# roncapat/UNIGE-TASI-path-planners

Hardware: AMD Instinct MI355X
Metric: grid cells updated/sec (full plan + 100 replans), 4096^2 map (higher is better)
Workload: dtype f32

## Files before the change

### unige-tasi-path-planners_amd/csrc/ufm_region.h

```cpp

#ifndef UFM_REGION_IDLE_SLEEP_RAISE
#define UFM_REGION_IDLE_SLEEP_RAISE 8
#endif
#ifndef UFM_REGION_PRIO
#define UFM_REGION_PRIO 2
#endif
#if UFM_REGION_PRIO
#define UFM_REGION_SETPRIO(x) __builtin_amdgcn_s_setprio(x)
#else
#define UFM_REGION_SETPRIO(x) do {} while (0)
#endif
#ifndef UFM_REGION_IDLE_SLEEP
#define UFM_REGION_IDLE_SLEEP 8
#endif
constexpr int RTMAX = 128 / T;
constexpr int RN = RTMAX * T;
constexpr int RP = RN + 8;
constexpr int RCP = RN + 4;
constexpr int RBP = RN;
constexpr int TP = T / 4;
constexpr int RPW = RTMAX * TP / 4;
constexpr int RWW = (RPW * RPW + 31) / 32;
constexpr int RFRAME = 4 * RTMAX + 4;

struct RegionJob {
    ReplanBegin rb;
    DevDyn dyn;
    int tx0, ty0, ntx, nty;
    int k_lower;
    unsigned int seq;
    int max_sweeps;
    int debug;
    float slack;
    float delta;
    int map;
    int batch;
    const uint8_t *psrc[4];
};
constexpr int RJOBS = 8;
struct RegionJobs { int n; RegionJob j[RJOBS]; };

__device__ __forceinline__ int prio_read_fresh(const DevParams &P, int qz, int kk, int gt) {
    const unsigned long long v = __hip_atomic_load(&P.prio[(size_t)(qz * 2 + (kk & 1)) * P.NT + gt], __ATOMIC_RELAXED, __HIP_MEMORY_SCOPE_AGENT);
    return (int)(v >> 32) == 0x7FFFFFFF - kk ? (int)(unsigned int)v : INFBITS;
}

struct RegionShared {
    int wake[16][RWW];
    int ever[16][RWW];
    int renew[16][RWW];
    int tbp[RTMAX * RTMAX];
    int seed[16][RWW];
    int defer[2][16][RWW];
    int dprio[2][RTMAX * RTMAX];
    int tflag[RTMAX * RTMAX];
    int traised[RTMAX * RTMAX];
    int actL[RFRAME], actR[RFRAME];
    int soff[4];
    float sdist[4];
    float B0, rbound;
    float theta;
    float Bgate;
    int rmin;
    float Bsub;
    int swas[4];
    int idle, giveup, again, any_start_in;
    unsigned long long sweeps;
    int expanded;
    int m_r, m_l, done;
    int dkey;
    int dbg[8];
    int dbg2[8];
    unsigned long long tstamp[12];
};

__device__ __forceinline__ float region_start_key(const float *Gs, const RegionShared &S) {
    if (!S.any_start_in) return S.B0;
    float b = 0.0f;
#pragma unroll
    for (int i = 0; i < 4; ++i) {
        const int o = S.soff[i];
        if (o < 0) continue;
        const float g = Gs[o];
        if (g < INFINITY) b = fmaxf(b, g + S.sdist[i]);
    }
    return b > 0.0f ? b : INFINITY;
}

__device__ __forceinline__ float region_lower_bound(const float *Gs, const RegionShared &S) {
    if (!S.any_start_in) return S.B0;
    float b = 0.0f;
    bool pending = false;
#pragma unroll
    for (int i = 0; i < 4; ++i) {
        const int o = S.soff[i];
        if (o < 0) continue;
        const float g = Gs[o];
        if (g < INFINITY) b = fmaxf(b, g + S.sdist[i]);
        else if (S.swas[i]) pending = true;
    }
    if (pending) return fmaxf(b, S.rbound);
    return b > 0.0f ? b : INFINITY;
}

template <int ALGOF, int MODE>
__device__ void region_phase(const DevParams &P, const RegionJob &J, float *Gs, const uint8_t *Cb, uint8_t *Bb, RegionShared &S,
                             int thr, float hm, int focused, int goal_lx, int goal_ly) {
    constexpr int ALGO = algo_of(ALGOF);
    constexpr bool FOLLOW = (ALGOF & ALGO_FOLLOW_INFO) != 0;
    constexpr bool BPRAISE = MODE == MODE_RAISE && (!is_dfm<ALGO> || FOLLOW);
    const int tid = threadIdx.x, w = wave_index16(tid >> 6), lane = tid & 63;
    const int q = lane & 3, nd = lane >> 2;
    const int nprow = J.ntx * TP, npcol = J.nty * TP;
    unsigned long long wake_sel = 0ull;
    if (lane < 9) {
        const int dr = lane / 3 - 1, dc = lane % 3 - 1;
        wake_sel = ~0ull;
        if (dr < 0) wake_sel &= 0x000000000000FFFFull; else if (dr > 0) wake_sel &= 0xFFFF000000000000ull;
        if (dc < 0) wake_sel &= 0x000F000F000F000Full; else if (dc > 0) wake_sel &= 0xF000F000F000F000ull;
    }
    const int colour = ((nd >> 2) & 1) | ((nd & 1) << 1);
    const bool wt_lane = lane < 9;
    const int wt_dr = wt_lane ? lane / 3 - 1 : 0, wt_dc = wt_lane ? lane % 3 - 1 : 0;
    const int wt_ar = (w >> 2) + wt_dr, wt_ac = (w & 3) + wt_dc;
    const int wt_wave = ((wt_ar & 3) << 2) | (wt_ac & 3), wt_di = (wt_ar >> 2) * RPW + (wt_ac >> 2);
    const float sx = J.rb.sb.sx, sy = J.rb.sb.sy;
    const int rx0 = J.tx0 * T, ry0 = J.ty0 * T;
    int budget = J.max_sweeps;
    unsigned int my_sweeps = 0;
    auto cost_at = [=](int r, int c) { const int b = Cb[r * RCP + c]; return b >= thr ? INFINITY : (float)b; };
    const int so0 = __builtin_amdgcn_readfirstlane(S.soff[0]), so1 = __builtin_amdgcn_readfirstlane(S.soff[1]);
    const int so2 = __builtin_amdgcn_readfirstlane(S.soff[2]), so3 = __builtin_amdgcn_readfirstlane(S.soff[3]);
    const bool dbg_nogate = (J.debug & 1) != 0, dbg_count = (J.debug & 2) != 0;
    const float Bphase = (MODE == MODE_LOWER) ? S.Bgate : INFINITY;
    const float rb_phase = S.rbound + J.slack;
    const int nwords = min(RWW, (((nprow + 3) / 4 - 1) * RPW + (npcol + 3) / 4 + 31) / 32);
    UFM_REGION_SETPRIO(UFM_REGION_PRIO);
    for (;;) {
        bool took = false;
        bool vote = __hip_atomic_load(&S.giveup, __ATOMIC_RELAXED, __HIP_MEMORY_SCOPE_WORKGROUP) != 0;
        for (int wd = 0; wd < nwords && !vote; ++wd) {
            if (__hip_atomic_load(&S.wake[w][wd], __ATOMIC_RELAXED, __HIP_MEMORY_SCOPE_WORKGROUP) == 0) continue;
            int bits = 0;
            if (lane == 0) bits = atomicExch(&S.wake[w][wd], 0);
            bits = __builtin_amdgcn_readfirstlane(bits);
            if (!bits) continue;
            if (MODE == MODE_RAISE && lane == 0) S.ever[w][wd] |= bits;
            int seedbits = 0;
            if (BPRAISE) seedbits = __builtin_amdgcn_readfirstlane(S.seed[w][wd]) & bits;
            while (bits) {
                const int j = __ffs(bits) - 1;
                if (budget <= 0) {
                    if (lane == 0) {
                        __hip_atomic_fetch_or(&S.wake[w][wd], bits, __ATOMIC_RELAXED, __HIP_MEMORY_SCOPE_WORKGROUP);
                        __hip_atomic_store(&S.giveup, 1, __ATOMIC_RELAXED, __HIP_MEMORY_SCOPE_WORKGROUP);
                    }
                    vote = true;
                    break;
                }
                bits &= bits - 1;
                took = true;
                const int idx = wd * 32 + j;
                const int pr = (idx / RPW) * 4 + (w >> 2), pc = (idx % RPW) * 4 + (w & 3);
                if (pr >= nprow || pc >= npcol) continue;
                const int lx = pr * 4 + (nd >> 2), ly = pc * 4 + (nd & 3);
                const bool arith = BPRAISE && ((seedbits >> j) & 1);
                QuadConsts<ALGO> C;
                if (!BPRAISE || arith) C.load_at(cost_at, lx, ly, q, RP);
                float *ctr = Gs + (lx + 1) * RP + ly + 1;
                uint8_t *bpp = Bb + lx * RBP + ly;
                const int bpb = BPRAISE ? *bpp : BP_NONE;
                const int bqc = bpb >> 3, bsx = (bqc & 2) ? RP : -RP, bsy = (bqc & 1) ? 1 : -1;
                int bo1 = (bpb & 4) ? bsy : bsx, bo2 = bsx + bsy;
                if constexpr (is_dfm<ALGO>) dfm_bp_offsets<RP>(bpb, bo1, bo2);
                const bool bd1 = bpb & 1, bd2 = bpb & 2;
                const bool bnone = is_dfm<ALGO> && bpb == BP_NONE;
                const bool goal = (lx == goal_lx) & (ly == goal_ly);
                const int npr = pr + wt_dr, npc = pc + wt_dc, ni = idx + wt_di;
                const bool wt_ok = wt_lane & ((unsigned)npr < (unsigned)nprow) & ((unsigned)npc < (unsigned)npcol);
                const int nwave = wt_wave, nword = wt_ok ? (ni >> 5) : -1, nbit = 1 << (ni & 31);
                float hd = 0.0f;
                if (hm != 0.0f) {
                    const float x0 = (float)(rx0 + pr * 4), x1 = x0 + 3.0f, y0 = (float)(ry0 + pc * 4), y1 = y0 + 3.0f;
                    const float dx = fmaxf(fmaxf(x0 - sx, sx - x1), 0.0f), dy = fmaxf(fmaxf(y0 - sy, sy - y1), 0.0f);
                    hd = hm * hypotf(dx, dy) * 0.999f;
                }
                const int tl = (pr / TP) * J.nty + (pc / TP);
                const float B = Bphase;
                const int my_off = (lx + 1) * RP + ly + 1;
                const bool is_start = (my_off == so0) | (my_off == so1) | (my_off == so2) | (my_off == so3);
                const float rb = (MODE == MODE_RAISE && S.traised[tl]) ? INFINITY : rb_phase;
                asm volatile("" ::: "memory");
                float g = ctr[0];
                if (dbg_count && MODE == MODE_LOWER) {
                    const int sx_ = (q & 2) ? RP : -RP, sy_ = (q & 1) ? 1 : -1;
                    const bool fin = (g < INFINITY) | (ctr[sx_] < INFINITY) | (ctr[sy_] < INFINITY) | (ctr[sx_ + sy_] < INFINITY);
                    if (__builtin_amdgcn_ballot_w64(fin) == 0ull && lane == 0) atomicAdd(&S.dbg2[1], 1);
                }
                float dmin = INFINITY;
                float rmin_l = INFINITY;
                bool again = true, pch = false;
                [[maybe_unused]] bool held_last = false;
                [[maybe_unused]] float nv_last = INFINITY;
                [[maybe_unused]] const bool gate_free = is_start || B == INFINITY || dbg_nogate;
                unsigned long long chg = 0ull;
                int cnt = 0;
                for (int b = 0; b < 16 && again; ++b) {
                    asm volatile("" ::: "memory");
                    float nv;
                    if constexpr (BPRAISE) {
                        if (arith && b == 0) nv = quad_min(eval_quad_bp<ALGO, RP>(ctr, q, C, bpb));
                        else { const float p1 = ctr[bo1], p2 = ctr[bo2]; nv = ((bd1 && p1 == INFINITY) || (bd2 && p2 == INFINITY) || bnone) ? INFINITY : g; }
                    }
                    else nv = quad_min(eval_quad<ALGO, RP>(ctr, q, C));
                    if (goal) nv = 0.0f;
                    bool want, gate, doit;
                    if (MODE == MODE_LOWER) {
                        want = (nv != g);
                        gate = (nv + hd < B) || gate_free;
                        doit = want && gate && ((nv < g) || (colour == (cnt & 3)));
                        held_last = want && !gate; nv_last = nv;
                    } else {
                        if (is_dfm<ALGO>) want = (g < INFINITY) && (nv > g) && ((nv == INFINITY) || (__float_as_int(nv) - __float_as_int(g) > 8));
                        else want = (g < INFINITY) && (nv > g);
                        gate = !(g > rb) || dbg_nogate;
                        doit = want && gate;
                        if (want && !gate) dmin = fminf(dmin, g);
                        rmin_l = doit ? fminf(rmin_l, g) : rmin_l;
                        nv = INFINITY;
                    }
                    if (doit && q == 0) ctr[0] = nv;
                    const float gn = doit ? nv : g;
                    const unsigned long long mask = __builtin_amdgcn_ballot_w64(doit);
                    const unsigned long long wanted = __builtin_amdgcn_ballot_w64(want && gate);
                    g = gn;
                    pch |= mask != 0ull;
                    chg |= mask;
                    UFM_SWEEP_FENCE();
                    if ((mask & wake_sel) != 0ull && nword >= 0 && lane != 4)
                        __hip_atomic_fetch_or(&S.wake[nwave][nword], nbit, __ATOMIC_RELAXED, __HIP_MEMORY_SCOPE_WORKGROUP);
                    ++cnt;
                    again = wanted != 0ull;
                }
                budget -= cnt; my_sweeps += cnt;
                if (pch && lane == 0) S.tflag[tl] = 1;
                if (MODE == MODE_LOWER && held_last) dmin = nv_last;
                if ((chg & wake_sel) != 0ull && nword >= 0) __hip_atomic_fetch_or(&S.renew[nwave][nword], nbit, __ATOMIC_RELAXED, __HIP_MEMORY_SCOPE_WORKGROUP);
                if (BPRAISE && arith) {
                    const unsigned long long held = __builtin_amdgcn_ballot_w64(dmin < INFINITY);
                    if (lane == 0 && held == 0ull) S.seed[w][wd] &= ~(1 << j);
                }
                if (MODE == MODE_RAISE && rmin_l < INFINITY && q == 0) { atomicMin(&S.rmin, __float_as_int(rmin_l)); S.traised[tl] = 1; }
                if (dbg_count && lane == 0) { atomicAdd(&S.dbg[MODE == MODE_LOWER ? 5 : 4], 1); atomicAdd(&S.dbg[MODE == MODE_LOWER ? 7 : 6], cnt); if (!pch) atomicAdd(&S.dbg2[MODE == MODE_LOWER ? 0 : 2], 1); }
                if (again && lane == 0) __hip_atomic_fetch_or(&S.wake[w][wd], 1 << j, __ATOMIC_RELAXED, __HIP_MEMORY_SCOPE_WORKGROUP);
                if (dmin < INFINITY && q == 0) {
                    atomicAdd(&S.dbg[MODE == MODE_LOWER ? 0 : 1], 1);
                    atomicMin(&S.dprio[MODE == MODE_LOWER ? 0 : 1][tl], __float_as_int(dmin));
                    if (MODE == MODE_LOWER) atomicMin(&S.dkey, __float_as_int(dmin + hd));
                    __hip_atomic_fetch_or(&S.defer[MODE == MODE_LOWER ? 0 : 1][w][wd], 1 << j, __ATOMIC_RELAXED, __HIP_MEMORY_SCOPE_WORKGROUP);
                }
            }
        }
        if (took && !vote) continue;
        if (!vote) {
            if (lane == 0) atomicAdd(&S.idle, 1);
            UFM_REGION_SETPRIO(0);
            for (;;) {
                __builtin_amdgcn_s_sleep(BPRAISE ? UFM_REGION_IDLE_SLEEP_RAISE : UFM_REGION_IDLE_SLEEP);
                const int idle_now = __hip_atomic_load(&S.idle, __ATOMIC_RELAXED, __HIP_MEMORY_SCOPE_WORKGROUP);
                const int gave_up_now = __hip_atomic_load(&S.giveup, __ATOMIC_RELAXED, __HIP_MEMORY_SCOPE_WORKGROUP);
                int any = 0;
#pragma unroll
                for (int wd = 0; wd < RWW; ++wd) any |= __hip_atomic_load(&S.wake[w][wd], __ATOMIC_RELAXED, __HIP_MEMORY_SCOPE_WORKGROUP);
                if (idle_now >= 16 || gave_up_now != 0) { vote = true; break; }
                if (any) { if (lane == 0) atomicSub(&S.idle, 1); break; }
            }
            UFM_REGION_SETPRIO(UFM_REGION_PRIO);
            if (!vote) continue;
        }
        __syncthreads();
        int mine = 0;
#pragma unroll
        for (int wd = 0; wd < RWW; ++wd) mine |= __hip_atomic_load(&S.wake[w][wd], __ATOMIC_RELAXED, __HIP_MEMORY_SCOPE_WORKGROUP);
        const int work = __syncthreads_or(mine != 0);
        const int gave_up = __hip_atomic_load(&S.giveup, __ATOMIC_RELAXED, __HIP_MEMORY_SCOPE_WORKGROUP);
        if (gave_up || !work) break;
        if (tid == 0) S.idle = 0;
        __syncthreads();
    }
    UFM_REGION_SETPRIO(0);
    if (lane == 0 && my_sweeps) atomicAdd(&S.sweeps, (unsigned long long)my_sweeps);
    __syncthreads();
    if (tid == 0) S.idle = 0;
    __syncthreads();
}

template <int ALGOF>
__global__ __launch_bounds__(NTHR) void k_replan_region(DevParams P, RegionJobs JS, DevCounters *host, unsigned int *flag) {
    constexpr int ALGO = algo_of(ALGOF);
    __shared__ float Gs[(RN + 2) * RP];
    __shared__ uint8_t Cb[(RN + 1) * RCP];
    __shared__ __attribute__((aligned(16))) uint8_t Bb[RN * RBP];
    __shared__ RegionShared S;
    __shared__ int s_last;
#ifdef UFM_REGION_NG0
    constexpr int NG0 = UFM_REGION_NG0;
#else
    constexpr int NG0 = (46 * 1024) / (TT * 4);
#endif
    __shared__ float G0c[NG0 * TT];
    __shared__ int s_wbl[RTMAX * RTMAX];
    __shared__ int s_nwb;
    __shared__ uint8_t s_pmask[4096];
    __shared__ int s_simd[16];
    __shared__ unsigned long long s_tb[8];
    constexpr bool CELLS = is_dfm<ALGO>;
    constexpr int COFF = CELLS ? 0 : 1;
    const int tid = threadIdx.x;
    const RegionJob &J = JS.j[blockIdx.x];
    const int m = J.map, gt0 = m * P.NTm;
    const int ntl = J.ntx * J.nty;
    const int nty_magic = (65536 + J.nty - 1) / J.nty;
    const int rx0 = J.tx0 * T, ry0 = J.ty0 * T, rnx = J.ntx * T, rny = J.nty * T;

    const unsigned long long t_begin = wall_clock64();
#define STAMP(k) do { if (tid == 0 && (J.debug & 2)) s_tb[k] = wall_clock64(); } while (0)
    STAMP(0);
    if ((tid & 63) == 0 && (J.debug & 2)) s_simd[tid >> 6] = (int)__builtin_amdgcn_s_getreg((1 << 11) | (4 << 6) | 4);
    const float hm = J.dyn.hm;
    const int thr = J.dyn.thr, focused = J.dyn.focused;
    int r_first = -1;
    for (int r = J.rb.nrect - 1; r >= 0; --r) if (J.psrc[r]) r_first = r;
    const bool one_fused = J.rb.nrect == 1 && r_first == 0 && !J.batch;
    int pb0[4] = {0, 0, 0, 0};
    if (r_first >= 0) {
        const int n0 = J.rb.rect[r_first][3] * J.rb.rect[r_first][4];
#pragma unroll
        for (int c = 0; c < 4; ++c) { const int e = tid + c * NTHR; if (e < n0) pb0[c] = J.psrc[r_first][e]; }
    }
    float sg = INFINITY;
    int se_x = -1, se_y = -1;
    {
        const int e = tid == 0 ? J.rb.sb.start[0] : (tid == 1 ? J.rb.sb.start[1] : (tid == 2 ? J.rb.sb.start[2] : (tid == 3 ? J.rb.sb.start[3] : -1)));
        if (e >= 0) { se_x = e / P.EY; se_y = e - se_x * P.EY; sg = P.G[gaddr(P, m, se_x, se_y)]; }
    }
    const int n_pending = P.ctr->scount;
    const int goal_x = P.goal[2 * m], goal_y = P.goal[2 * m + 1];
    STAMP(1);
    const int wv = __builtin_amdgcn_readfirstlane(tid >> 6), ln = tid & 63;
    {
        const int crow = rnx + COFF, ccol = rny + COFF;
        constexpr int KP = (RN + 64) / 64, KR = (RN + 16) / 16;
        const uint8_t *cbase = P.cost + (size_t)m * P.cstride;
        uint8_t cv[KP * KR];
#pragma unroll
        for (int j = 0; j < KP; ++j) {
            const int c = j * 64 + ln, cy = ry0 + c - COFF;
            const bool cok = c < ccol && cy >= 0 && cy < P.W;
#pragma unroll
            for (int k = 0; k < KR; ++k) {
                const int r = wv + 16 * k, cx = rx0 + r - COFF;
                cv[j * KR + k] = 255;
                if (j * 64 < ccol && r < crow && cx >= 0 && cx < P.L && cok) cv[j * KR + k] = cbase[(size_t)cx * P.W + cy];
            }
        }
        constexpr int CPT = TT / 256, KT = RTMAX * RTMAX * CPT / 16;
        float4 gv[KT];
        unsigned int bv[KT];
#pragma unroll
        for (int k = 0; k < KT; ++k) {
            const int pc = wv + 16 * k, tl = pc / CPT;
            if (tl >= ntl) continue;
            const int ti = (tl * nty_magic) >> 16, tj = tl - ti * J.nty, v = (pc - tl * CPT) * 64 + ln;
            const size_t gt = (size_t)(gt0 + (J.tx0 + ti) * P.TY + J.ty0 + tj);
            gv[k] = reinterpret_cast<const float4 *>(P.G + gt * TT)[v];
            bv[k] = reinterpret_cast<const unsigned int *>(P.bp + gt * TT)[v];
        }
        static_assert(4 * RN + 4 <= NTHR, "one frame element per thread");
        float fv = INFINITY;
        int fo = -1;
        if (tid < 2 * (rny + 2) + 2 * rnx) {
            int hx, hy;
            if (tid < rny + 2) { hx = -1; hy = tid - 1; }
            else if (tid < 2 * (rny + 2)) { hx = rnx; hy = tid - (rny + 2) - 1; }
            else if (tid < 2 * (rny + 2) + rnx) { hx = tid - 2 * (rny + 2); hy = -1; }
            else { hx = tid - 2 * (rny + 2) - rnx; hy = rny; }
            const int x = rx0 + hx, y = ry0 + hy;
            fo = (hx + 1) * RP + hy + 1;
            if (x >= 0 && y >= 0 && x < P.TX * T && y < P.TY * T) fv = P.G[gaddr(P, m, x, y)];
        }
        STAMP(7);
#pragma unroll
        for (int j = 0; j < KP; ++j) {
            const int c = j * 64 + ln;
#pragma unroll
            for (int k = 0; k < KR; ++k) {
                const int r = wv + 16 * k;
                if (j * 64 < ccol && r < crow && c < ccol) Cb[r * RCP + c] = cv[j * KR + k];
            }
        }
#pragma unroll
        for (int k = 0; k < KT; ++k) {
            const int pc = wv + 16 * k, tl = pc / CPT;
            if (tl >= ntl) continue;
            const int ti = (tl * nty_magic) >> 16, tj = tl - ti * J.nty, e = ((pc - tl * CPT) * 64 + ln) * 4;
            float *g = &Gs[(ti * T + e / T + 1) * RP + tj * T + e % T + 1];
            g[0] = gv[k].x; g[1] = gv[k].y; g[2] = gv[k].z; g[3] = gv[k].w;
            *reinterpret_cast<unsigned int *>(&Bb[(ti * T + e / T) * RBP + tj * T + e % T]) = bv[k];
        }
        if (fo >= 0) Gs[fo] = fv;
    }
    for (int r = 0; r < J.rb.nrect; ++r) {
        if (!J.psrc[r]) continue;
        const int *qr = J.rb.rect[r];
        const int px = qr[1], py = qr[2], pw = qr[3], ph = qr[4];
        const unsigned pw_magic = ((1u << 20) + (unsigned)pw - 1u) / (unsigned)pw;
        __syncthreads();
        STAMP(2);
#pragma unroll
        for (int c = 0; c < 4; ++c) {
            const int e = tid + c * NTHR;
            if (e >= pw * ph) continue;
            const int i = (int)(((unsigned)e * pw_magic) >> 20), j = e - i * pw;
            uint8_t *cb = &Cb[(px + i - rx0 + COFF) * RCP + (py + j - ry0 + COFF)];
            const uint8_t nv = (r == r_first) ? (uint8_t)pb0[c] : J.psrc[r][e];
            const uint8_t ch = *cb != nv;
            s_pmask[e] = ch;
            if (ch) { *cb = nv; P.cost[(size_t)m * P.cstride + (size_t)(px + i) * P.W + (py + j)] = nv; cost_window_store(P, m, px + i, py + j, nv); }
        }
        __syncthreads();
        STAMP(3);
        const int ne = CELLS ? pw * ph : (pw + 1) * (ph + 1);
        if (one_fused) {
            const int ew = CELLS ? pw : pw + 1;
            const unsigned ew_magic = ((1u << 20) + (unsigned)ew - 1u) / (unsigned)ew;
            int cnt = 0;
            for (int e = tid; e < ne; e += NTHR) {
                const int i = (int)(((unsigned)e * ew_magic) >> 20), j = e - i * ew;
                bool ch;
                if (!CELLS) ch = (i > 0 && j > 0 && s_pmask[(i - 1) * pw + j - 1]) || (i > 0 && j < pw && s_pmask[(i - 1) * pw + j]) ||
                                 (i < ph && j > 0 && s_pmask[i * pw + j - 1]) || (i < ph && j < pw && s_pmask[i * pw + j]);
                else ch = s_pmask[i * pw + j];
                cnt += ch ? 1 : 0;
            }
            for (int o = 32; o; o >>= 1) cnt += __shfl_xor(cnt, o);
            if ((tid & 63) == 0 && cnt) atomicAdd(&P.num_updated[m], (unsigned int)cnt);
        } else {
            for (int base = 0; base < ne; base += NTHR) patch_seed<!CELLS>(P, m, s_pmask, px, py, pw, ph, base + tid);
        }
    }
    if (J.rb.nrect && J.psrc[J.rb.nrect - 1]) __syncthreads();
    STAMP(4);
    if (tid == 0 && !J.batch) *P.dyn = J.dyn;
    if (!J.batch) step_begin(P, J.rb.sb);
    if (!one_fused)
        for (int r = 0; r < J.rb.nrect; ++r) {
            const int *qr = J.rb.rect[r];
            for (int e = tid; e < (qr[3] + 1) * (qr[4] + 1); e += NTHR) clear_mark(P, qr[0], qr[1], qr[2], qr[3], qr[4], e);
        }
    for (int i = tid; i < (int)(sizeof(RegionShared) / sizeof(int)); i += NTHR) reinterpret_cast<int *>(&S)[i] = 0;
    __syncthreads();
    STAMP(5);
    for (int i = tid; i < 2 * RTMAX * RTMAX; i += NTHR) (&S.dprio[0][0])[i] = INFBITS;
    for (int i = tid; i < RFRAME; i += NTHR) { S.actL[i] = INFBITS; S.actR[i] = INFBITS; }
    if (tid == 0) { S.rmin = INFBITS; S.m_r = INFBITS; }
    {
        const int n = one_fused ? n_pending : P.ctr->scount;
        for (int i = tid; i < n; i += NTHR) {
            const int gt = P.slist[i];
            if (gt / P.NTm != m) continue;
            const int tx = (gt - gt0) / P.TY, ty = (gt - gt0) - tx * P.TY;
            P.sflag[gt] = 0;
            if (tx < J.tx0 || tx >= J.tx0 + J.ntx || ty < J.ty0 || ty >= J.ty0 + J.nty) activate(P, Q_RAISE, J.rb.k_raise, gt, 0);
        }
        __syncthreads();
        STAMP(6);
        if (tid == 0 && !J.batch) { P.ctr->scount = 0; P.ctr->done = 0; }
        if (tid < 64) {
            float key = 0.0f, dist = 0.0f;
            int off = -1;
            if (se_x >= 0) {
                dist = hm * hypotf(J.rb.sb.sx - (float)se_x, J.rb.sb.sy - (float)se_y);
                if (sg < INFINITY) key = sg + dist;
                if (se_x >= rx0 && se_x < rx0 + rnx && se_y >= ry0 && se_y < ry0 + rny) off = (se_x - rx0 + 1) * RP + (se_y - ry0 + 1);
            }
            if (tid < 4) { S.soff[tid] = off; S.sdist[tid] = dist; }
            const bool in = __builtin_amdgcn_ballot_w64(off >= 0) != 0ull;
            float b0 = fmaxf(key, __shfl_xor(key, 1));
            b0 = fmaxf(b0, __shfl_xor(b0, 2));
            if (tid == 0) {
                b0 = b0 > 0.0f ? b0 : INFINITY;
                S.B0 = b0;
                S.rbound = focused ? b0 + J.rb.band : INFINITY;
                S.any_start_in = in ? 1 : 0;
            }
        }
    }

    if (tid == 0) { S.tstamp[0] = t_begin; S.tstamp[1] = wall_clock64(); S.tstamp[2] = S.tstamp[1]; }
    __syncthreads();
    for (int r = 0; r < J.rb.nrect; ++r) {
        const int *qr = J.rb.rect[r];
        const int ex0 = qr[1] - rx0, ex1 = qr[1] + qr[4] - (CELLS ? 1 : 0) - rx0, ey0 = qr[2] - ry0, ey1 = qr[2] + qr[3] - (CELLS ? 1 : 0) - ry0;
        const int p0 = max(ex0, 0) / 4, p1 = min(ex1, rnx - 1) / 4, c0 = max(ey0, 0) / 4, c1 = min(ey1, rny - 1) / 4;
        const int np = (p1 - p0 + 1) * (c1 - c0 + 1);
        for (int i = tid; i < np; i += NTHR) {
            const int pr = p0 + i / (c1 - c0 + 1), pc = c0 + i % (c1 - c0 + 1);
            const int ni = (pr >> 2) * RPW + (pc >> 2);
            atomicOr(&S.wake[((pr & 3) << 2) | (pc & 3)][ni >> 5], 1 << (ni & 31));
            atomicOr(&S.seed[((pr & 3) << 2) | (pc & 3)][ni >> 5], 1 << (ni & 31));
            S.traised[(pr / TP) * J.nty + pc / TP] = 1;
        }
    }
    if (tid < 4) S.swas[tid] = (S.soff[tid] >= 0 && Gs[S.soff[tid]] < INFINITY) ? 1 : 0;
    __syncthreads();
    const int goal_lx = goal_x - rx0, goal_ly = goal_y - ry0;

    for (int round = 0;; ++round) {
        for (;;) {
            region_phase<ALGOF, MODE_RAISE>(P, J, Gs, Cb, Bb, S, thr, hm, focused, goal_lx, goal_ly);
            const int again_t = __syncthreads_or(tid < ntl && S.traised[tid] && S.dprio[1][tid] != INFBITS) && !S.giveup;
            __syncthreads();
            if (!again_t) break;
            for (int i = tid; i < 16 * RWW; i += NTHR) { (&S.wake[0][0])[i] |= (&S.defer[1][0][0])[i]; (&S.defer[1][0][0])[i] = 0; }
            for (int i = tid; i < RTMAX * RTMAX; i += NTHR) S.dprio[1][i] = INFBITS;
            __syncthreads();
        }
        if (tid == 0 && round == 0) S.tstamp[3] = wall_clock64();
        for (int i = tid; i < 16 * RWW; i += NTHR) {
            (&S.wake[0][0])[i] |= (&S.ever[0][0])[i] | (&S.defer[0][0][0])[i];
            (&S.ever[0][0])[i] = 0; (&S.defer[0][0][0])[i] = 0;
        }
        for (int i = tid; i < RTMAX * RTMAX; i += NTHR) S.dprio[0][i] = INFBITS;
        if (tid == 0) {
            S.dkey = INFBITS;
            S.Bsub = focused ? region_lower_bound(Gs, S) : INFINITY;
            S.theta = (round == 0) ? ((S.rmin != INFBITS) ? __int_as_float(S.rmin) + J.delta : INFINITY) : S.theta;
            S.Bgate = fminf(S.Bsub + J.slack, S.theta);
        }
        __syncthreads();
        for (int sub = 0;; ++sub) {
            region_phase<ALGO, MODE_LOWER>(P, J, Gs, Cb, Bb, S, thr, hm, focused, goal_lx, goal_ly);
            if (tid == 0) {
                const float B = focused ? region_lower_bound(Gs, S) : INFINITY;
                const int m = S.dkey;
                bool again = !S.giveup && m != INFBITS && (__int_as_float(m) < B || B == INFINITY);
                if (again && sub >= 4096) { again = false; S.giveup = 1; }
                S.again = again ? 1 : 0;
                S.Bsub = B;
                if (again) S.theta = fmaxf(S.theta, __int_as_float(m)) + J.delta;
                S.Bgate = fminf(S.Bsub + J.slack, S.theta);
            }
            __syncthreads();
            const int again_l = S.again;
            __syncthreads();
            if (!again_l) break;
            if (tid == 0) ++S.dbg[2];
            for (int i = tid; i < 16 * RWW; i += NTHR) { (&S.wake[0][0])[i] |= (&S.defer[0][0][0])[i]; (&S.defer[0][0][0])[i] = 0; }
            for (int i = tid; i < RTMAX * RTMAX; i += NTHR) S.dprio[0][i] = INFBITS;
            if (tid == 0) S.dkey = INFBITS;
            __syncthreads();
        }
        if (tid < ntl && S.dprio[1][tid] != INFBITS) atomicMin(&S.m_r, S.dprio[1][tid]);
        __syncthreads();
        if (tid == 0) {
            const float B = focused ? region_lower_bound(Gs, S) : INFINITY;
            const int m = S.m_r;
            S.m_r = INFBITS;
            bool again = !S.giveup && focused && m != INFBITS && __int_as_float(m) < B + J.slack;
            if (again && round >= 14) { again = false; S.giveup = 1; }
            if (again) S.rbound = fmaxf(B, S.rbound) + J.rb.band;
            S.again = again ? 1 : 0;
        }
        __syncthreads();
        const int again_r = S.again;
        __syncthreads();
        if (!again_r) break;
        if (tid == 0) ++S.dbg[3];
        for (int i = tid; i < 16 * RWW; i += NTHR) { (&S.wake[0][0])[i] |= (&S.defer[1][0][0])[i]; (&S.defer[1][0][0])[i] = 0; }
        for (int i = tid; i < RTMAX * RTMAX; i += NTHR) S.dprio[1][i] = INFBITS;
        __syncthreads();
    }

    {
        const int w = wave_index16(tid >> 6), lane = tid & 63, q = lane & 3, nd = lane >> 2;
        const int nprow = J.ntx * TP, npcol = J.nty * TP;
        auto cost_at = [=](int r, int c) { const int b = Cb[r * RCP + c]; return b >= thr ? INFINITY : (float)b; };
        for (int wd = 0; wd < RWW; ++wd) {
            int bits = __builtin_amdgcn_readfirstlane(S.renew[w][wd]);
            while (bits) {
                const int j = __ffs(bits) - 1;
                bits &= bits - 1;
                const int idx = wd * 32 + j;
                const int pr = (idx / RPW) * 4 + (w >> 2), pc = (idx % RPW) * 4 + (w & 3);
                if (pr >= nprow || pc >= npcol) continue;
                const int lx = pr * 4 + (nd >> 2), ly = pc * 4 + (nd & 3);
                QuadConsts<ALGO> C;
                C.load_at(cost_at, lx, ly, q, RP);
                const LaneEval le = eval_quad_w<ALGO, RP>(Gs + (lx + 1) * RP + ly + 1, q, C);
                const float nv = quad_min(le.r);
                const int bq = quad_min_int(bp_byte<ALGO>(le, q, C, le.r == nv)), b = bp_of_key<ALGO>(bq);
                if (q == 0) Bb[lx * RBP + ly] = (uint8_t)((lx == goal_lx && ly == goal_ly) ? BP_NONE : b);
                if (lane == 0) S.tbp[(pr / TP) * J.nty + pc / TP] = 1;
            }
        }
        __syncthreads();
    }
    if (tid == 0) S.tstamp[4] = wall_clock64();
    auto frame_index = [&](int ti, int tj) {
        if (ti < 0) return tj + 1;
        if (ti >= J.ntx) return (J.nty + 2) + tj + 1;
        if (tj < 0) return 2 * (J.nty + 2) + ti;
        return 2 * (J.nty + 2) + J.ntx + ti;
    };
    static_assert(NTHR == 1024 && TT % 64 == 0 && RBP % 4 == 0, "the block kernel deals its staging and write-back out by wave");
    constexpr int UPT = TT / 64;
    const int wvw = __builtin_amdgcn_readfirstlane(tid >> 6), lnw = tid & 63;
    if (tid < 64) {
        const bool has = tid < ntl && (S.tflag[tid] | S.tbp[tid]);
        const unsigned long long hm_ = __builtin_amdgcn_ballot_w64(has);
        if (has) s_wbl[__popcll(hm_ & ((1ull << tid) - 1ull))] = tid;
        if (tid == 0) s_nwb = __popcll(hm_);
    }
    __syncthreads();
    const int nunits = s_nwb * UPT;
    auto unit_tile = [&](int u, int &k, int &part, int &tl, int &ti, int &tj) {
        k = u / UPT; part = u - k * UPT; tl = __builtin_amdgcn_readfirstlane(s_wbl[k]);
        ti = (tl * nty_magic) >> 16; tj = tl - ti * J.nty;
    };
    {
        typedef __attribute__((address_space(3))) void *lds_ptr;
        typedef const __attribute__((address_space(1))) void *glb_ptr;
#pragma unroll 1
        for (int u = wvw; u < nunits; u += 16) {
            int k, part, tl, ti, tj;
            unit_tile(u, k, part, tl, ti, tj);
            if (!S.tflag[tl] || k >= NG0) continue;
            const size_t gt = (size_t)(gt0 + (J.tx0 + ti) * P.TY + J.ty0 + tj);
            __builtin_amdgcn_global_load_lds((glb_ptr)(P.G + gt * TT + part * 64 + lnw), (lds_ptr)(G0c + k * TT + part * 64), 4, 0, 0);
        }
        asm volatile("s_waitcnt vmcnt(0)" ::: "memory");
    }
    __syncthreads();
    int n_exp = 0;
#pragma unroll 1
    for (int u = wvw; u < nunits; u += 16) {
        int k, part, tl, ti, tj;
        unit_tile(u, k, part, tl, ti, tj);
        const int e = part * 64 + lnw;
        if (S.tbp[tl]) P.bp[(size_t)(gt0 + (J.tx0 + ti) * P.TY + J.ty0 + tj) * TT + e] = Bb[(ti * T + e / T) * RBP + tj * T + e % T];
        if (!S.tflag[tl]) continue;
        const int tx = J.tx0 + ti, ty = J.ty0 + tj, gt = gt0 + tx * P.TY + ty;
        const int io_r = e / T, io_c = e % T;
        float gl0;
        if (k < NG0) gl0 = G0c[k * TT + e];
        else { gl0 = P.G[(size_t)gt * TT + e]; P.Gprev[(size_t)gt * TT + e] = gl0; }
        const float gf = Gs[(ti * T + io_r + 1) * RP + tj * T + io_c + 1];
        if (gf == gl0) continue;
        ++n_exp;
        P.G[(size_t)gt * TT + e] = gf;
        const int er = (io_r == 0) ? -1 : ((io_r == T - 1) ? 1 : 0);
        const int ec = (io_c == 0) ? -1 : ((io_c == T - 1) ? 1 : 0);
        const bool rok = er && tx + er >= 0 && tx + er < P.TX, cok = ec && ty + ec >= 0 && ty + ec < P.TY;
        if (rok) P.ring[(size_t)(gt + er * P.TY) * RING + (er < 0 ? RING_BOT : RING_TOP) + io_c] = gf;
        if (cok) P.ring[(size_t)(gt + ec) * RING + (ec < 0 ? RING_RIGHT : RING_LEFT) + io_r] = gf;
        if (rok && cok) P.ring[(size_t)(gt + er * P.TY + ec) * RING + RING_CORNER + (er < 0 ? 2 : 0) + (ec < 0 ? 1 : 0)] = gf;
        const bool out_r = rok && (ti + er < 0 || ti + er >= J.ntx), out_c = cok && (tj + ec < 0 || tj + ec >= J.nty);
        if (!(out_r || out_c)) continue;
        const int lxr = ti * T + io_r + 1, lyc = tj * T + io_c + 1;
        const int cl = max(io_c - 1, 0) - io_c, ch = min(io_c + 1, T - 1) - io_c;
        const int rl = max(io_r - 1, 0) - io_r, rh = min(io_r + 1, T - 1) - io_r;
        const float lo = fminf(gf, gl0);
        const bool lowered = gf < gl0;
        const int pb = __float_as_int(lowered ? gf : gl0);
        auto concerned = [&](float a, float b, float c) {
            if (lowered) return lo < fmaxf(fmaxf(a, b), c);
            const float fa = a < INFINITY ? a : -INFINITY, fb = b < INFINITY ? b : -INFINITY, fc = c < INFINITY ? c : -INFINITY;
            return gl0 < fmaxf(fmaxf(fa, fb), fc);
        };
        if (out_r) {
            const float *h = Gs + (lxr + er) * RP + lyc;
            if (concerned(h[cl], h[0], h[ch])) atomicMin(lowered ? &S.actL[frame_index(ti + er, tj)] : &S.actR[frame_index(ti + er, tj)], pb);
        }
        if (out_c) {
            const float *h = Gs + lxr * RP + lyc + ec;
            if (concerned(h[rl * RP], h[0], h[rh * RP])) atomicMin(lowered ? &S.actL[frame_index(ti, tj + ec)] : &S.actR[frame_index(ti, tj + ec)], pb);
        }
        if (rok && cok && (out_r || out_c)) {
            const int di = ti + er, dj = tj + ec;
            if (di < 0 || di >= J.ntx || dj < 0 || dj >= J.nty) {
                const float hv = Gs[(lxr + er) * RP + lyc + ec];
                if (concerned(hv, hv, hv)) atomicMin(lowered ? &S.actL[frame_index(di, dj)] : &S.actR[frame_index(di, dj)], pb);
            }
        }
    }
    if (n_exp) atomicAdd(&S.expanded, n_exp);
    __syncthreads();
    for (int i = tid; i < 2 * (J.nty + 2) + 2 * J.ntx; i += NTHR) {
        int ti, tj;
        if (i < J.nty + 2) { ti = -1; tj = i - 1; }
        else if (i < 2 * (J.nty + 2)) { ti = J.ntx; tj = i - (J.nty + 2) - 1; }
        else if (i < 2 * (J.nty + 2) + J.ntx) { ti = i - 2 * (J.nty + 2); tj = -1; }
        else { ti = i - 2 * (J.nty + 2) - J.ntx; tj = J.nty; }
        const int tx = J.tx0 + ti, ty = J.ty0 + tj;
        if (tx < 0 || ty < 0 || tx >= P.TX || ty >= P.TY) continue;
        const int gt = gt0 + tx * P.TY + ty;
        if (S.actR[i] != INFBITS) activate(P, Q_RAISE, J.rb.k_raise, gt, S.actR[i]);
        if (S.actL[i] != INFBITS) activate(P, Q_LOWER, J.k_lower, gt, S.actL[i]);
    }
    for (int tl = tid; tl < ntl; tl += NTHR) {
        const int gt = gt0 + (J.tx0 + tl / J.nty) * P.TY + J.ty0 + tl % J.nty;
        if (S.dprio[0][tl] != INFBITS) park_tile(P, Q_LOWER, gt, S.dprio[0][tl]);
        if (S.dprio[1][tl] != INFBITS) park_tile(P, Q_RAISE, gt, S.dprio[1][tl]);
    }
    if (S.giveup) {
        for (int i = tid; i < 16 * RWW * 32; i += NTHR) {
            const int w = i / (RWW * 32), r = i % (RWW * 32);
            if (!(S.wake[w][r >> 5] & (1 << (r & 31)))) continue;
            const int pr = (r / RPW) * 4 + (w >> 2), pc = (r % RPW) * 4 + (w & 3);
            if (pr >= J.ntx * TP || pc >= J.nty * TP) continue;
            const int gt = gt0 + (J.tx0 + pr / TP) * P.TY + J.ty0 + pc / TP;
            activate(P, Q_RAISE, J.rb.k_raise, gt, 0);
            activate(P, Q_LOWER, J.k_lower, gt, 0);
        }
    }
    if (J.batch) __threadfence(); else __builtin_amdgcn_fence(__ATOMIC_RELEASE, "workgroup");
    __syncthreads();

    if (tid == 0) S.tstamp[5] = wall_clock64();
    if (tid == 0) { S.m_r = INFBITS; S.m_l = INFBITS; }
    __syncthreads();
    {
        const float B = focused ? region_start_key(Gs, S) : INFINITY;
        int mr = INFBITS, ml = INFBITS;
        const int nr = __hip_atomic_load(&P.ctr->cnt[Q_RAISE][J.rb.k_raise % 3], __ATOMIC_RELAXED, __HIP_MEMORY_SCOPE_AGENT);
        const int npr = __hip_atomic_load(&P.ctr->npark[Q_RAISE], __ATOMIC_RELAXED, __HIP_MEMORY_SCOPE_AGENT);
        const int nl = __hip_atomic_load(&P.ctr->cnt[Q_LOWER][J.k_lower % 3], __ATOMIC_RELAXED, __HIP_MEMORY_SCOPE_AGENT);
        const int npl = __hip_atomic_load(&P.ctr->npark[Q_LOWER], __ATOMIC_RELAXED, __HIP_MEMORY_SCOPE_AGENT);
        auto mine = [&](int gt) { return (unsigned)gt < (unsigned)P.NT && gt / P.NTm == m; };
        for (int i = tid; i < nr; i += NTHR) {
            const int gt = __hip_atomic_load(&P.cand[(size_t)(Q_RAISE * 3 + J.rb.k_raise % 3) * P.NT + i], __ATOMIC_RELAXED, __HIP_MEMORY_SCOPE_AGENT);
            if (mine(gt)) mr = min(mr, prio_read_fresh(P, Q_RAISE, J.rb.k_raise, gt));
        }
        for (int i = tid; i < npr; i += NTHR) {
            const int gt = __hip_atomic_load(&P.park[(size_t)(Q_RAISE * 2) * P.NT + i], __ATOMIC_RELAXED, __HIP_MEMORY_SCOPE_AGENT);
            if (mine(gt)) mr = min(mr, __hip_atomic_load(&P.pprio[Q_RAISE * P.NT + gt], __ATOMIC_RELAXED, __HIP_MEMORY_SCOPE_AGENT));
        }
        auto lower_key = [&](int gt, int pbits) {
            if (pbits == INFBITS) return INFINITY;
            return __int_as_float(pbits) + (focused ? tile_heuristic(P, m, (gt - gt0) / P.TY, (gt - gt0) % P.TY) : 0.0f);
        };
        float kl = INFINITY;
        for (int i = tid; i < nl; i += NTHR) {
            const int gt = __hip_atomic_load(&P.cand[(size_t)(Q_LOWER * 3 + J.k_lower % 3) * P.NT + i], __ATOMIC_RELAXED, __HIP_MEMORY_SCOPE_AGENT);
            if (mine(gt)) kl = fminf(kl, lower_key(gt, prio_read_fresh(P, Q_LOWER, J.k_lower, gt)));
        }
        for (int i = tid; i < npl; i += NTHR) {
            const int gt = __hip_atomic_load(&P.park[(size_t)(Q_LOWER * 2) * P.NT + i], __ATOMIC_RELAXED, __HIP_MEMORY_SCOPE_AGENT);
            if (mine(gt)) kl = fminf(kl, lower_key(gt, __hip_atomic_load(&P.pprio[Q_LOWER * P.NT + gt], __ATOMIC_RELAXED, __HIP_MEMORY_SCOPE_AGENT)));
        }
        ml = kl < INFINITY ? __float_as_int(kl) : INFBITS;
        if (mr != INFBITS) atomicMin(&S.m_r, mr);
        if (ml != INFBITS) atomicMin(&S.m_l, ml);
        __syncthreads();
        if (tid == 0) {
            bool done;
            if (focused && B < INFINITY) done = !(__int_as_float(S.m_r) < B) && !(__int_as_float(S.m_l) < B);
            else done = (S.m_r == INFBITS && S.m_l == INFBITS) && (J.batch || (nr == 0 && nl == 0));
            if (S.giveup) done = false;
            S.done = done ? 1 : 0;
            unsigned int upd = 0;
            if (P.consume[m]) { upd = P.num_updated[m]; P.num_updated[m] = 0; }
            if (!J.batch) {
                P.ctr->done = S.done;
                P.ctr->rbound = S.rbound;
                P.ctr->qmin[Q_RAISE] = S.m_r;
                P.ctr->updated = upd;
                P.ctr->tile_visits += (unsigned long long)ntl;
                P.ctr->raise_visits += (unsigned long long)ntl / 2;
                P.ctr->tile_iters += S.sweeps / 16;
                P.ctr->elem_evals += 16ull * S.sweeps;
                if (done) P.ctr->expanded = (unsigned long long)S.expanded;
            } else {
                if (!done) atomicAdd(&P.ctr->done_fail, 1);
                if (S.m_r != INFBITS && __int_as_float(S.m_r) < S.rbound) atomicMin(&P.ctr->qmin[Q_RAISE], 0);
                atomicMax(reinterpret_cast<int *>(&P.ctr->rbound), __float_as_int(S.rbound));
                atomicAdd(&P.ctr->updated, upd);
                atomicAdd(&P.ctr->tile_visits, (unsigned long long)ntl);
                atomicAdd(&P.ctr->raise_visits, (unsigned long long)ntl / 2);
                atomicAdd(&P.ctr->tile_iters, S.sweeps / 16);
                atomicAdd(&P.ctr->elem_evals, 16ull * S.sweeps);
                if (done) atomicAdd(&P.ctr->expanded, (unsigned long long)S.expanded);
            }
            if (J.debug & 2) {
                int nd0 = 0, nd1 = 0, m0 = INFBITS, m1 = INFBITS;
                for (int i = 0; i < ntl; ++i) { if (S.dprio[0][i] != INFBITS) { ++nd0; m0 = min(m0, S.dprio[0][i]); } if (S.dprio[1][i] != INFBITS) { ++nd1; m1 = min(m1, S.dprio[1][i]); } }
                int *d = P.lmax;
                d[0] = __float_as_int(B); d[1] = __float_as_int(S.B0); d[2] = __float_as_int(S.rbound); d[3] = S.m_r; d[4] = S.m_l;
                d[5] = nr; d[6] = nl; d[7] = npr; d[8] = npl; d[9] = S.done; d[10] = S.giveup; d[11] = (int)S.sweeps; d[12] = S.expanded;
                d[13] = nd0; d[14] = m0; d[15] = nd1; d[16] = m1; d[17] = S.any_start_in;
                for (int i = 0; i < 4; ++i) d[18 + i] = S.soff[i] >= 0 ? __float_as_int(Gs[S.soff[i]]) : -1;
                for (int i = 0; i < 8; ++i) d[22 + i] = S.dbg[i];
                S.tstamp[6] = wall_clock64();
                for (int i = 1; i < 7; ++i) d[30 + i] = (int)(S.tstamp[i] - S.tstamp[0]);
                for (int i = 1; i < 8; ++i) d[40 + i] = (int)(s_tb[i] - s_tb[0]);
                for (int i = 0; i < 16; ++i) d[50 + i] = s_simd[i];
                for (int i = 0; i < 8; ++i) d[70 + i] = S.dbg2[i];
            }
        }
        __syncthreads();
    }
    if (!S.done) {
#pragma unroll 1
        for (int u = wvw; u < nunits; u += 16) {
            int k, part, tl, ti, tj;
            unit_tile(u, k, part, tl, ti, tj);
            if (!S.tflag[tl]) continue;
            const int e = part * 64 + lnw;
            const int gt = gt0 + (J.tx0 + ti) * P.TY + J.ty0 + tj;
            if (k < NG0) P.Gprev[(size_t)gt * TT + e] = G0c[k * TT + e];
            if (e == 0) {
                P.fresh[gt] = 0;
                if (atomicAdd(&P.touched[gt], 1) == 0) P.tlist[atomicAdd(&P.ctr->tcount, 1)] = gt;
            }
        }
    }
    if (J.batch) __threadfence();
    __syncthreads();
    if (J.batch) {
        if (tid == 0) s_last = (atomicAdd(&P.ctr->fin_blocks, 1) == (int)gridDim.x - 1);
        __syncthreads();
        if (!s_last) return;
        __threadfence();
        if (tid == 0) {
            P.ctr->fin_blocks = 0;
            P.ctr->scount = 0;
            P.ctr->done = __hip_atomic_load(&P.ctr->done_fail, __ATOMIC_RELAXED, __HIP_MEMORY_SCOPE_AGENT) == 0 ? 1 : 0;
        }
        __threadfence();
        __syncthreads();
    }
    const int *src = reinterpret_cast<const int *>(P.ctr);
    int *dst = reinterpret_cast<int *>(host);
    for (int i = tid; i < (int)(sizeof(DevCounters) / sizeof(int)); i += NTHR)
        dst[i] = __hip_atomic_load(&src[i], __ATOMIC_RELAXED, __HIP_MEMORY_SCOPE_AGENT);
    __syncthreads();
    if (tid == 0) __hip_atomic_store(flag, J.seq, __ATOMIC_RELEASE, __HIP_MEMORY_SCOPE_SYSTEM);
}
```

Measured before the change: 572.7 million.

## Hoist region shared-state init and seeding earlier, stage G0 snapshot during load

Moves the RegionShared initialization (zero/INF fill in one pass), the step_begin call, the start-key computation and the wake/seed bit marking ahead of the patch loop, so several __syncthreads barriers can be dropped. When the region fits in NG0 tiles, the initial G snapshot is written into G0c straight from the registers already loaded, which skips the later global_load_lds copy and its barrier. It also reads consume/num_updated before the final reduction barrier. This reorders when shared state is written relative to the patch step, and it relies on later code not depending on the old ordering.

Result: no change. 573.7 million, median of 4 (+0.2%).

```diff
diff --git a/unige-tasi-path-planners_amd/csrc/ufm_region.h b/unige-tasi-path-planners_amd/csrc/ufm_region.h
--- a/unige-tasi-path-planners_amd/csrc/ufm_region.h
+++ b/unige-tasi-path-planners_amd/csrc/ufm_region.h
@@ -308,7 +308,7 @@
 #else
     constexpr int NG0 = (46 * 1024) / (TT * 4);
 #endif
-    __shared__ float G0c[NG0 * TT];
+    __shared__ __attribute__((aligned(16))) float G0c[NG0 * TT];
     __shared__ int s_wbl[RTMAX * RTMAX];
     __shared__ int s_nwb;
     __shared__ uint8_t s_pmask[4096];
@@ -390,6 +390,18 @@
             if (x >= 0 && y >= 0 && x < P.TX * T && y < P.TY * T) fv = P.G[gaddr(P, m, x, y)];
         }
         STAMP(7);
+        if (tid == 0 && !J.batch) *P.dyn = J.dyn;
+        if (!J.batch) step_begin(P, J.rb.sb);
+        {
+            constexpr int o_dprio = (int)(offsetof(RegionShared, dprio) / sizeof(int)), o_act = (int)(offsetof(RegionShared, actL) / sizeof(int));
+            constexpr int o_rmin = (int)(offsetof(RegionShared, rmin) / sizeof(int)), o_mr = (int)(offsetof(RegionShared, m_r) / sizeof(int));
+            static_assert(offsetof(RegionShared, actR) == offsetof(RegionShared, actL) + RFRAME * sizeof(int), "actL and actR are filled as one range");
+            for (int i = tid; i < (int)(sizeof(RegionShared) / sizeof(int)); i += NTHR) {
+                const bool inf = (unsigned)(i - o_dprio) < 2u * RTMAX * RTMAX || (unsigned)(i - o_act) < 2u * RFRAME || i == o_rmin || i == o_mr;
+                reinterpret_cast<int *>(&S)[i] = inf ? INFBITS : 0;
+            }
+        }
+        STAMP(5);
 #pragma unroll
         for (int j = 0; j < KP; ++j) {
             const int c = j * 64 + ln;
@@ -406,16 +418,50 @@
             const int ti = (tl * nty_magic) >> 16, tj = tl - ti * J.nty, e = ((pc - tl * CPT) * 64 + ln) * 4;
             float *g = &Gs[(ti * T + e / T + 1) * RP + tj * T + e % T + 1];
             g[0] = gv[k].x; g[1] = gv[k].y; g[2] = gv[k].z; g[3] = gv[k].w;
+            if (!CELLS && ntl <= NG0) *reinterpret_cast<float4 *>(&G0c[tl * TT + e]) = gv[k];
             *reinterpret_cast<unsigned int *>(&Bb[(ti * T + e / T) * RBP + tj * T + e % T]) = bv[k];
         }
         if (fo >= 0) Gs[fo] = fv;
+    }
+    __syncthreads();
+    if (tid < 64) {
+        float key = 0.0f, dist = 0.0f;
+        int off = -1;
+        if (se_x >= 0) {
+            dist = hm * hypotf(J.rb.sb.sx - (float)se_x, J.rb.sb.sy - (float)se_y);
+            if (sg < INFINITY) key = sg + dist;
+            if (se_x >= rx0 && se_x < rx0 + rnx && se_y >= ry0 && se_y < ry0 + rny) off = (se_x - rx0 + 1) * RP + (se_y - ry0 + 1);
+        }
+        if (tid < 4) { S.soff[tid] = off; S.sdist[tid] = dist; S.swas[tid] = (off >= 0 && Gs[off] < INFINITY) ? 1 : 0; }
+        const bool in = __builtin_amdgcn_ballot_w64(off >= 0) != 0ull;
+        float b0 = fmaxf(key, __shfl_xor(key, 1));
+        b0 = fmaxf(b0, __shfl_xor(b0, 2));
+        if (tid == 0) {
+            b0 = b0 > 0.0f ? b0 : INFINITY;
+            S.B0 = b0;
+            S.rbound = focused ? b0 + J.rb.band : INFINITY;
+            S.any_start_in = in ? 1 : 0;
+        }
+    }
+    for (int r = 0; r < J.rb.nrect; ++r) {
+        const int *qr = J.rb.rect[r];
+        const int ex0 = qr[1] - rx0, ex1 = qr[1] + qr[4] - (CELLS ? 1 : 0) - rx0, ey0 = qr[2] - ry0, ey1 = qr[2] + qr[3] - (CELLS ? 1 : 0) - ry0;
+        const int p0 = max(ex0, 0) / 4, p1 = min(ex1, rnx - 1) / 4, c0 = max(ey0, 0) / 4, c1 = min(ey1, rny - 1) / 4;
+        const int np = (p1 - p0 + 1) * (c1 - c0 + 1);
+        for (int i = tid; i < np; i += NTHR) {
+            const int pr = p0 + i / (c1 - c0 + 1), pc = c0 + i % (c1 - c0 + 1);
+            const int ni = (pr >> 2) * RPW + (pc >> 2);
+            atomicOr(&S.wake[((pr & 3) << 2) | (pc & 3)][ni >> 5], 1 << (ni & 31));
+            atomicOr(&S.seed[((pr & 3) << 2) | (pc & 3)][ni >> 5], 1 << (ni & 31));
+            S.traised[(pr / TP) * J.nty + pc / TP] = 1;
+        }
     }
     for (int r = 0; r < J.rb.nrect; ++r) {
         if (!J.psrc[r]) continue;
         const int *qr = J.rb.rect[r];
         const int px = qr[1], py = qr[2], pw = qr[3], ph = qr[4];
         const unsigned pw_magic = ((1u << 20) + (unsigned)pw - 1u) / (unsigned)pw;
-        __syncthreads();
+        if (r != r_first) __syncthreads();
         STAMP(2);
 #pragma unroll
         for (int c = 0; c < 4; ++c) {
@@ -451,19 +497,11 @@
     }
     if (J.rb.nrect && J.psrc[J.rb.nrect - 1]) __syncthreads();
     STAMP(4);
-    if (tid == 0 && !J.batch) *P.dyn = J.dyn;
-    if (!J.batch) step_begin(P, J.rb.sb);
     if (!one_fused)
         for (int r = 0; r < J.rb.nrect; ++r) {
             const int *qr = J.rb.rect[r];
             for (int e = tid; e < (qr[3] + 1) * (qr[4] + 1); e += NTHR) clear_mark(P, qr[0], qr[1], qr[2], qr[3], qr[4], e);
         }
-    for (int i = tid; i < (int)(sizeof(RegionShared) / sizeof(int)); i += NTHR) reinterpret_cast<int *>(&S)[i] = 0;
-    __syncthreads();
-    STAMP(5);
-    for (int i = tid; i < 2 * RTMAX * RTMAX; i += NTHR) (&S.dprio[0][0])[i] = INFBITS;
-    for (int i = tid; i < RFRAME; i += NTHR) { S.actL[i] = INFBITS; S.actR[i] = INFBITS; }
-    if (tid == 0) { S.rmin = INFBITS; S.m_r = INFBITS; }
     {
         const int n = one_fused ? n_pending : P.ctr->scount;
         for (int i = tid; i < n; i += NTHR) {
@@ -476,44 +514,8 @@
         __syncthreads();
         STAMP(6);
         if (tid == 0 && !J.batch) { P.ctr->scount = 0; P.ctr->done = 0; }
-        if (tid < 64) {
-            float key = 0.0f, dist = 0.0f;
-            int off = -1;
-            if (se_x >= 0) {
-                dist = hm * hypotf(J.rb.sb.sx - (float)se_x, J.rb.sb.sy - (float)se_y);
-                if (sg < INFINITY) key = sg + dist;
-                if (se_x >= rx0 && se_x < rx0 + rnx && se_y >= ry0 && se_y < ry0 + rny) off = (se_x - rx0 + 1) * RP + (se_y - ry0 + 1);
-            }
-            if (tid < 4) { S.soff[tid] = off; S.sdist[tid] = dist; }
-            const bool in = __builtin_amdgcn_ballot_w64(off >= 0) != 0ull;
-            float b0 = fmaxf(key, __shfl_xor(key, 1));
-            b0 = fmaxf(b0, __shfl_xor(b0, 2));
-            if (tid == 0) {
-                b0 = b0 > 0.0f ? b0 : INFINITY;
-                S.B0 = b0;
-                S.rbound = focused ? b0 + J.rb.band : INFINITY;
-                S.any_start_in = in ? 1 : 0;
-            }
-        }
-    }
-
+    }
     if (tid == 0) { S.tstamp[0] = t_begin; S.tstamp[1] = wall_clock64(); S.tstamp[2] = S.tstamp[1]; }
-    __syncthreads();
-    for (int r = 0; r < J.rb.nrect; ++r) {
-        const int *qr = J.rb.rect[r];
-        const int ex0 = qr[1] - rx0, ex1 = qr[1] + qr[4] - (CELLS ? 1 : 0) - rx0, ey0 = qr[2] - ry0, ey1 = qr[2] + qr[3] - (CELLS ? 1 : 0) - ry0;
-        const int p0 = max(ex0, 0) / 4, p1 = min(ex1, rnx - 1) / 4, c0 = max(ey0, 0) / 4, c1 = min(ey1, rny - 1) / 4;
-        const int np = (p1 - p0 + 1) * (c1 - c0 + 1);
-        for (int i = tid; i < np; i += NTHR) {
-            const int pr = p0 + i / (c1 - c0 + 1), pc = c0 + i % (c1 - c0 + 1);
-            const int ni = (pr >> 2) * RPW + (pc >> 2);
-            atomicOr(&S.wake[((pr & 3) << 2) | (pc & 3)][ni >> 5], 1 << (ni & 31));
-            atomicOr(&S.seed[((pr & 3) << 2) | (pc & 3)][ni >> 5], 1 << (ni & 31));
-            S.traised[(pr / TP) * J.nty + pc / TP] = 1;
-        }
-    }
-    if (tid < 4) S.swas[tid] = (S.soff[tid] >= 0 && Gs[S.soff[tid]] < INFINITY) ? 1 : 0;
-    __syncthreads();
     const int goal_lx = goal_x - rx0, goal_ly = goal_y - ry0;
 
     for (int round = 0;; ++round) {
@@ -628,7 +630,8 @@
         k = u / UPT; part = u - k * UPT; tl = __builtin_amdgcn_readfirstlane(s_wbl[k]);
         ti = (tl * nty_magic) >> 16; tj = tl - ti * J.nty;
     };
-    {
+    const bool copy_staged = !CELLS && ntl <= NG0;
+    if (!copy_staged) {
         typedef __attribute__((address_space(3))) void *lds_ptr;
         typedef const __attribute__((address_space(1))) void *glb_ptr;
 #pragma unroll 1
@@ -640,8 +643,8 @@
             __builtin_amdgcn_global_load_lds((glb_ptr)(P.G + gt * TT + part * 64 + lnw), (lds_ptr)(G0c + k * TT + part * 64), 4, 0, 0);
         }
         asm volatile("s_waitcnt vmcnt(0)" ::: "memory");
-    }
-    __syncthreads();
+        __syncthreads();
+    }
     int n_exp = 0;
 #pragma unroll 1
     for (int u = wvw; u < nunits; u += 16) {
@@ -653,7 +656,8 @@
         const int tx = J.tx0 + ti, ty = J.ty0 + tj, gt = gt0 + tx * P.TY + ty;
         const int io_r = e / T, io_c = e % T;
         float gl0;
-        if (k < NG0) gl0 = G0c[k * TT + e];
+        const int ci = copy_staged ? tl : k;
+        if (ci < NG0) gl0 = G0c[ci * TT + e];
         else { gl0 = P.G[(size_t)gt * TT + e]; P.Gprev[(size_t)gt * TT + e] = gl0; }
         const float gf = Gs[(ti * T + io_r + 1) * RP + tj * T + io_c + 1];
         if (gf == gl0) continue;
@@ -737,6 +741,8 @@
         const int npr = __hip_atomic_load(&P.ctr->npark[Q_RAISE], __ATOMIC_RELAXED, __HIP_MEMORY_SCOPE_AGENT);
         const int nl = __hip_atomic_load(&P.ctr->cnt[Q_LOWER][J.k_lower % 3], __ATOMIC_RELAXED, __HIP_MEMORY_SCOPE_AGENT);
         const int npl = __hip_atomic_load(&P.ctr->npark[Q_LOWER], __ATOMIC_RELAXED, __HIP_MEMORY_SCOPE_AGENT);
+        const int consume_m = __hip_atomic_load(&P.consume[m], __ATOMIC_RELAXED, __HIP_MEMORY_SCOPE_AGENT);
+        const unsigned int updated_m = __hip_atomic_load(&P.num_updated[m], __ATOMIC_RELAXED, __HIP_MEMORY_SCOPE_AGENT);
         auto mine = [&](int gt) { return (unsigned)gt < (unsigned)P.NT && gt / P.NTm == m; };
         for (int i = tid; i < nr; i += NTHR) {
             const int gt = __hip_atomic_load(&P.cand[(size_t)(Q_RAISE * 3 + J.rb.k_raise % 3) * P.NT + i], __ATOMIC_RELAXED, __HIP_MEMORY_SCOPE_AGENT);
@@ -770,7 +776,7 @@
             if (S.giveup) done = false;
             S.done = done ? 1 : 0;
             unsigned int upd = 0;
-            if (P.consume[m]) { upd = P.num_updated[m]; P.num_updated[m] = 0; }
+            if (consume_m) { upd = updated_m; P.num_updated[m] = 0; }
             if (!J.batch) {
                 P.ctr->done = S.done;
                 P.ctr->rbound = S.rbound;
@@ -818,7 +824,8 @@
             if (!S.tflag[tl]) continue;
             const int e = part * 64 + lnw;
             const int gt = gt0 + (J.tx0 + ti) * P.TY + J.ty0 + tj;
-            if (k < NG0) P.Gprev[(size_t)gt * TT + e] = G0c[k * TT + e];
+            const int ci = copy_staged ? tl : k;
+            if (ci < NG0) P.Gprev[(size_t)gt * TT + e] = G0c[ci * TT + e];
             if (e == 0) {
                 P.fresh[gt] = 0;
                 if (atomicAdd(&P.touched[gt], 1) == 0) P.tlist[atomicAdd(&P.ctr->tcount, 1)] = gt;
```
